# arielgabizon/barretenberg

Measured on AMD Instinct MI355X. Metric: BN254 G1 MSM points/sec at n=2^20 (Fr NTT elems/sec in 'ntt'), higher is better.
Workload: dtype u32x9 (256-bit Montgomery, 29-bit limbs)

## Files before the change

### barretenberg_amd/bbgpu.py

```python
import ctypes as C
import os
import subprocess

import numpy as np

try:
    import torch
except Exception:
    torch = None

HERE = os.path.dirname(os.path.abspath(__file__))
os.environ.setdefault("GPU_MAX_HW_QUEUES", "16")
u64p = C.POINTER(C.c_uint64)

NTT_KINDS = {
    "fft": 0,
    "ifft": 1,
    "coset_fft": 2,
    "coset_ifft": 3,
    "fft_with_constant": 4,
    "ifft_with_constant": 5,
    "coset_fft_with_constant": 6,
}

C_ABI_SYMBOLS = [
    "bbgpu_init", "bbgpu_shutdown", "bbgpu_device_count", "bbgpu_last_error", "bbgpu_version", "bbgpu_ntt",
    "bbgpu_ntt_device", "bbgpu_ntt_device_batch", "bbgpu_srs_register", "bbgpu_srs_release", "bbgpu_srs_generate", "bbgpu_srs_generate_range", "bbgpu_set_precompute",
    "bbgpu_srs_num_windows", "bbgpu_transcript_read_g1", "bbgpu_transcript_write", "bbgpu_msm_g1", "bbgpu_msm_g1_plain",
    "bbgpu_msm_g1_batch", "bbgpu_msm_num_windows", "bbgpu_msm_g1_device", "bbgpu_msm_g1_device_async", "bbgpu_msm_g1_device_rows_async", "bbgpu_msm_g1_device_buckets_async", "bbgpu_srs_has_window_tables", "bbgpu_msm_g1_wait",
    "bbgpu_msm_g1_device_batch_async", "bbgpu_msm_g1_batch_wait",
    "bbgpu_g1_sum", "bbgpu_last_timing", "bbgpu_set_host_thresholds", "bbgpu_srs_cache_stats", "bbgpu_set_table_share", "bbgpu_set_point_share", "bbgpu_selftest_field", "bbgpu_selftest_g1",
    "bbgpu_set_timing",
    "bbgpu_fr_evaluate_device", "bbgpu_fr_batch_invert_device", "bbgpu_fr_product_scan_device", "bbgpu_fr_mul_device",
    "bbgpu_kate_opening_device", "bbgpu_lagrange_l1_fft_device", "bbgpu_divide_by_pseudo_vanishing_device",
    "bbgpu_permutation_lagrange_base_device",
    "bbgpu_fr_evaluate", "bbgpu_kate_opening", "bbgpu_lagrange_l1_fft", "bbgpu_divide_by_pseudo_vanishing", "bbgpu_lagrange_evaluations",
    "bbgpu_generate_point_table",
    "bbgpu_plonk_prover_create", "bbgpu_plonk_prover_set_witness", "bbgpu_plonk_construct_proof", "bbgpu_plonk_preprocess", "bbgpu_plonk_last_challenges",
    "bbgpu_plonk_last_timing", "bbgpu_plonk_prover_destroy", "bbgpu_plonk_challenges_from_proof",
    "bbgpu_plonk_construct_proof_batch", "bbgpu_plonk_batch_challenges", "bbgpu_plonk_last_batch_timing",
    "bbgpu_host_msm_g1", "bbgpu_host_ntt", "bbgpu_host_fr_evaluate", "bbgpu_host_kate_opening", "bbgpu_host_lagrange_l1_fft",
    "bbgpu_host_divide_by_pseudo_vanishing", "bbgpu_memory_stats", "bbgpu_fault_inject", "bbgpu_fault_stats", "bbgpu_srs_set_validate",
    "bbgpu_init_devices", "bbgpu_num_contexts", "bbgpu_memory_stats_context",
    "bbgpu_plonk_check_witness", "bbgpu_plonk_check_witness_batch", "bbgpu_plonk_set_witness_check", "bbgpu_plonk_last_witness_report",
    "bbgpu_host_plonk_check_witness",
    "bbgpu_plonk_prover_set_wire_map", "bbgpu_plonk_prover_set_witness_from", "bbgpu_plonk_construct_proof_batch_from",
# ... 240 lines not shown
        arr = (MsmJob * len(jobs))()
        for j, (pts, sc, n) in zip(arr, jobs):
            j.points, j.scalars, j.num_elements = _ptr(pts), _ptr(sc), n
        self._chk(self.lib.bbgpu_msm_g1_batch(arr, len(jobs)))
        return [np.array(list(j.output), dtype=np.uint64) for j in arr]

    def msm_num_windows(self, n):
        return int(self.lib.bbgpu_msm_num_windows(n))

    def srs_num_windows(self, handle, n):
        return self._chk(self.lib.bbgpu_srs_num_windows(handle, n))

    def set_host_thresholds(self, msm_max_points, ntt_max_elements):
        self.lib.bbgpu_set_host_thresholds(int(msm_max_points), int(ntt_max_elements))

    def set_table_share(self, rank, world):
        self.lib.bbgpu_set_table_share(int(rank), int(world))

    def set_point_share(self, world):
        self.lib.bbgpu_set_point_share(int(world))

    def set_precompute(self, on=True):
        self.lib.bbgpu_set_precompute(1 if on else 0)

    def msm_device(self, handle, d_scalars_ptr, n, offset=0, window_begin=0, window_end=None, stream=None):
        if window_end is None:
            window_end = self.srs_num_windows(handle, n)
        out = np.zeros(12, dtype=np.uint64)
        self._chk(self.lib.bbgpu_msm_g1_device(handle, offset, C.c_void_p(d_scalars_ptr), n, window_begin, window_end,
                                               _ptr(out), C.c_void_p(stream or 0)))
# ... 106 lines not shown
```

### barretenberg_amd/csrc/bbgpu_internal.h

```cpp
#pragma once
#include <hip/hip_runtime.h>
#include <stddef.h>
#include <stdint.h>

#include <mutex>

#include "../../include/bbgpu.h"

namespace bbgpu {

void set_error(const char* fmt, ...);

hipError_t dev_malloc(void** p, size_t bytes);
hipError_t dev_free(void* p);
hipError_t h2d_async(void* dst, const void* src, size_t bytes, hipStream_t st);
hipError_t d2h_async(void* dst, const void* src, size_t bytes, hipStream_t st);
hipError_t launch_check();
struct DevBuf {
    void* p = nullptr;
    DevBuf() = default;
    DevBuf(const DevBuf&) = delete;
    DevBuf& operator=(const DevBuf&) = delete;
    ~DevBuf() { if (p) (void)dev_free(p); }
    template <class T> T* as() const { return static_cast<T*>(p); }
// ... 12 lines not shown
    int count = 0;
    float ms[8];
};
struct MsmWorkspace {
    uint8_t* base = nullptr;
    size_t cap = 0;
    void* h_out = nullptr;
    static size_t bytes_needed(size_t n, int c, int nw, int ng = 0);
    int ensure(size_t bytes);
    void release();
};
struct MsmPiece {
    uint32_t c = 0, nw = 0, wb = 0, hbits = 0, lbits = 0;
    uint32_t hout_group = 0;
    bool trivial = false;
};
struct AccRing {
    static constexpr int SIZE = 8;
    hipEvent_t end[SIZE] = {};
    uint64_t seq = 0;
    void release();
};
constexpr int MSM_MAX_JOBS = 4;
constexpr int MSM_MAX_PIECES = 64;
constexpr uint32_t MSM_HOUT_GROUPS = 256;
struct MsmSlot {
    MsmWorkspace ws;
    MsmPiece piece[MSM_MAX_PIECES];
    int npieces = 0;
    bool append = false;
    int helper = -1;
    bool is_helper = false;
    bool reserved = false;
    hipStream_t stream = nullptr;
    hipEvent_t done = nullptr;
    hipEvent_t ev[8] = { nullptr, nullptr, nullptr, nullptr, nullptr, nullptr, nullptr, nullptr };
    bool pending = false, trivial = false, timed = false, timed_light = false;
    size_t n = 0;
    uint32_t jobs = 1;
    uint64_t acc_seq = 0;
    AccRing* acc_ring = nullptr;
    bool throughput = false;
    void release();
};
int msm_choose_c(size_t n);
int msm_num_windows(int c);
int msm_issue(MsmSlot& S, const uint32_t* d_srs, const uint32_t* d_tab, size_t tab_stride, int tab_c, const uint64_t* d_scalars, size_t n, int wb,
              int we, hipStream_t st, int want_timing);
int msm_issue_batch(MsmSlot& S, const uint32_t* d_srs, const uint32_t* d_tab, size_t tab_stride, int tab_c, const uint64_t* const* d_scalars_v, int jobs,
                    size_t n, int wb, int we, hipStream_t st, int want_timing, uint32_t row_i0 = 0, uint32_t row_i1 = 0xffffffffu, uint32_t brow0 = 0,
                    uint32_t brow1 = 0xffffffffu);
int msm_issue_buckets(MsmSlot& S, const uint32_t* d_srs, const uint32_t* d_tab, size_t tab_stride, int tab_c, const uint64_t* d_scalars, size_t n,
                      uint32_t share, uint32_t share_count, hipStream_t st, int want_timing);
int msm_issue_rows(MsmSlot& S, const uint32_t* d_srs, const uint32_t* d_tab, size_t tab_stride, int tab_c, const uint64_t* d_scalars, size_t n,
                   uint64_t row_begin, uint64_t row_end, hipStream_t st, int want_timing);
int msm_finish_batch(MsmSlot& S, host::Xyzz* results, MsmTiming* timing);
int srs_build_table(const uint32_t* d_srs, size_t n, int c, int num_windows, int w_begin, int w_end, uint32_t** d_alloc_out, uint32_t** d_tab_out, hipStream_t st);
int msm_finish(MsmSlot& S, host::Xyzz* result, MsmTiming* timing);
int srs_upload(const uint64_t* host_table, size_t n, uint32_t** d_srs_out, hipStream_t st, size_t stride_bytes = 128);
int srs_upload_into(const uint64_t* host_table, size_t n, uint32_t* d_raw, uint32_t* d_srs, hipStream_t st, size_t stride_bytes);
int srs_generate(const uint64_t* x_mont256, size_t first, size_t n, uint32_t** d_srs_out, uint64_t* host_table_out, hipStream_t st);

int host_to_device(void* d_dst, const void* h_src, size_t bytes, hipStream_t st);
int device_to_host_sync(void* h_dst, const void* d_src, size_t bytes, hipStream_t st, bool* touched = nullptr);
void host_stage_release();
int bind_calling_thread();

std::mutex& plonk_mutex();
void plonk_release_all_locked();
uint64_t plonk_lane_bytes();

// ... 2 lines not shown
```

### barretenberg_amd/csrc/capi.hip

```cpp
#include <hip/hip_runtime.h>

#include <algorithm>
#include <mutex>
#include <stdarg.h>
#include <stdio.h>
#include <stdlib.h>
#include <string.h>
#include <time.h>
#include <atomic>
#include <condition_variable>
#include <exception>
#include <functional>
#include <thread>
#include <unordered_map>
#include <vector>

#include "bbgpu_internal.h"
#include "host_g1.hpp"
#include "host_g2.hpp"
#include "host_small.hpp"
#include "host_fallback.hpp"
#include "host_copy_pool.hpp"
#include "multi_plan.hpp"
#include "poly.h"
// ... 786 lines not shown
    SrsEntry& e = ctx().srs[idx];
    if (trace_srs()) fprintf(stderr, "bbgpu srs: full check: contents of %p differ from the resident copy\n", (const void*)e.host_ptr);
    if (e.auto_registered) free_entry(e);
    else e.stale_for_host = true;
}

int log2_exact(size_t n)
{
    if (n == 0 || (n & (n - 1))) return -1;
    int l = 0;
    while (((size_t)1 << l) < n) l++;
    return l;
}

int msm_host_ptrs_once(const uint64_t* scalars, const uint64_t* points, size_t n, host::Xyzz* out, bool plain, bool* stale);
int msm_host_ptrs_sum(const uint64_t* scalars, const uint64_t* points, size_t n, host::Xyzz* out, bool plain = false)
{
    bool stale = false;
    int rc = msm_host_ptrs_once(scalars, points, n, out, plain, &stale);
    if (stale) rc = msm_host_ptrs_once(scalars, points, n, out, plain, &stale);
    return rc;
}
int msm_host_ptrs(const uint64_t* scalars, const uint64_t* points, size_t n, uint64_t out[12], bool plain = false)
{
    host::Xyzz res;
    const int rc = msm_host_ptrs_sum(scalars, points, n, &res, plain);
    if (rc == BBGPU_OK) host::g1_to_normalised(res, out);
    return rc;
}
int msm_host_ptrs_once(const uint64_t* scalars, const uint64_t* points, size_t n, host::Xyzz* out, bool plain, bool* stale)
// ... 68 lines not shown
    const SrsEntry& e = is_transient ? transient : ctx().srs[idx];
    static const size_t split_env = [] { const char* v = getenv("BBGPU_HOST_MSM_SPLIT"); return v ? (size_t)std::max(1, atoi(v)) : (size_t)0; }();
    struct Range { size_t o, len; };
    std::vector<Range> ranges;
    {
        PointPiece pc[MAX_POINT_PIECES];
        const int np = split_pieces(e, off, n, pc, MAX_POINT_PIECES);
        if (np < 0) {
            if (is_transient && !small_once) (void)dev_free(transient.d_srs);
            set_error("MSM of %zu points spans more than %d table segments", n, MAX_POINT_PIECES);
            return BBGPU_ERR_SIZE;
        }
        if (np > 1) {
            for (int k = 0; k < np; k++) ranges.push_back(Range{ pc[k].first, pc[k].len });
        } else {
            const size_t parts = ns < 2 ? 1 : (split_env ? split_env : (n >= ((size_t)1 << 19) ? 2 : 1));
            const size_t base = parts == 2 ? ((n * 3 / 8) & ~(size_t)7) : n / parts;
            for (size_t k = 0; k < parts; k++) {
                const size_t o = k * base, len = (k + 1 == parts) ? n - o : base;
                if (len) ranges.push_back(Range{ o, len });
            }
        }
    }
    size_t max_len = 0;
    for (const auto& r : ranges) max_len = std::max(max_len, r.len);
    const double q1 = tr ? now_ms() : 0;
    uint64_t** stage[2] = { &ctx().d_stage, &ctx().d_stage2 };
    size_t* cap[2] = { &ctx().stage_cap, &ctx().stage2_cap };
    host::Xyzz res = host::g1_infinity();
    int rc = BBGPU_OK;
    size_t issued = 0, finished = 0;
    auto finish = [&](size_t k) -> int {
        host::Xyzz part;
        int r = finish_ticket(sl[k % (size_t)ns], &part, k + 1 == ranges.size() ? &ctx().last : nullptr);
        finished = k + 1;
        if (r == BBGPU_OK) res = host::g1_add(res, part);
        return r;
    };
    for (size_t k = 0; k < ranges.size() && rc == BBGPU_OK; k++) {
        const size_t w = k % (size_t)ns;
        if (k >= (size_t)ns) rc = finish(k - (size_t)ns);
        MsmSlot& S = ctx().slot[sl[w]];
        if (rc == BBGPU_OK) rc = grow(stage[w], cap[w], max_len * 32);
        if (rc == BBGPU_OK) rc = host_to_device(*stage[w], scalars + ranges[k].o * 4, ranges[k].len * 32, S.stream);
        if (rc == BBGPU_OK) rc = issue_on_entry(sl[w], e, off + ranges[k].o, *stage[w], ranges[k].len, 0, entry_windows(e, ranges[k].len), S.stream);
        if (rc == BBGPU_OK) issued = k + 1;
    }
    const double q2 = tr ? now_ms() : 0;
    if (rc == BBGPU_OK && full_check && !(bg.posted ? full_check_join(bg) : contents_match_full(ctx().srs[idx], off, points, n))) {
        for (int k = 0; k < ns; k++) drain_ticket(sl[k]);
        srs_mark_stale(idx);
        *stale = true;
        return BBGPU_OK;
    }
    while (rc == BBGPU_OK && finished < issued) rc = finish(finished);
    if (rc != BBGPU_OK) {
        char keep[sizeof(g_err)];
        memcpy(keep, g_err, sizeof(keep));
        for (int k = 0; k < ns; k++) drain_ticket(sl[k]);
        memcpy(g_err, keep, sizeof(keep));
    }
    const double q3 = tr ? now_ms() : 0;
    if (is_transient && !small_once) (void)dev_free(transient.d_srs);
    if (rc) return rc;
    *out = res;
    if (tr) fprintf(stderr, "bbgpu msm n=%zu: table %.3f, upload + issue %.3f, wait + host sums %.3f, free %.3f ms\n", n, q1 - q0, q2 - q1, q3 - q2, now_ms() - q3);
    return BBGPU_OK;
}

struct MultiWorker {
    std::mutex mu;
    std::condition_variable cv;
    std::function<int()> job;
    bool busy = false, stop = false;
    int rc = BBGPU_OK;
    std::exception_ptr ex;
    char err[sizeof(g_err)] = "";
    std::thread th;
    explicit MultiWorker(int k) { th = std::thread([this, k] { loop(k); }); }
    void loop(int k)
// ... 918 lines not shown
{
    std::lock_guard<std::recursive_mutex> lk(g_mu);
    return msm_host_ptrs(scalars, points, n, out, true);
}

void bbgpu_set_host_thresholds(int msm_max_points, int ntt_max_elements)
{
    std::lock_guard<std::recursive_mutex> lk(g_mu);
    for (auto& C : g_ctxs) {
        C.host_env_read = true;
        C.host_msm_max = msm_max_points < 0 ? 0 : msm_max_points;
        C.host_ntt_max = ntt_max_elements < 0 ? 0 : std::min(64, ntt_max_elements);
    }
}

static int msm_g1_batch_once(bbgpu_msm_job* jobs, size_t num_jobs, bool* stale, host::Xyzz* sums);
static int msm_g1_batch_run(bbgpu_msm_job* jobs, size_t num_jobs, host::Xyzz* sums)
{
    bool stale = false;
    int rc = msm_g1_batch_once(jobs, num_jobs, &stale, sums);
    if (stale) rc = msm_g1_batch_once(jobs, num_jobs, &stale, sums);
    return rc;
}
static bool batch_one_by_one(size_t n, int* sl)
{
    return n == 0 || n <= (size_t)ctx().host_msm_max || n > ((size_t)1 << 20) || free_slots(sl, 2) < 2;
}
static int msm_g1_batch_split(bbgpu_msm_job* jobs, size_t num_jobs, const multi::Slice* sl, int m)
{
    if (num_jobs == 0) return BBGPU_OK;
// ... 359 lines not shown
```

### barretenberg_amd/csrc/msm.hip

```cpp
#include <hip/hip_runtime.h>

#include <algorithm>
#include <mutex>
#include <stdint.h>
#include <stdio.h>
#include <stdlib.h>
#include <string.h>
#include <vector>

#include "bbgpu_internal.h"
#include "g1.hpp"
#include "g1_quad.hpp"
#include "host_g1.hpp"

namespace bbgpu {

using Fr = FrP;
#define FRONT_PRIO() __builtin_amdgcn_s_setprio(2)
constexpr int TAIL_PRIO = 3;
constexpr int SCALAR_BITS = 254;
constexpr int MSM_MAX_C = 16;
constexpr int MSM_THREADS = 256;

__device__ __forceinline__ void ld8(const uint32_t* p, uint32_t (&w)[8])
// ... 821 lines not shown
        if (t < half) {
            Xyzz q, r;
#pragma unroll
            for (int i = 0; i < NL; i++) {
                q.x.d[i] = sh[(0 * NL + i) * STRIDE + t];
                q.y.d[i] = sh[(1 * NL + i) * STRIDE + t];
                q.zz.d[i] = sh[(2 * NL + i) * STRIDE + t];
                q.zzz.d[i] = sh[(3 * NL + i) * STRIDE + t];
            }
            add(r, acc, q);
            acc = r;
        }
        __syncthreads();
    }
}
__global__ void __launch_bounds__(MSM_THREADS) TAIL_OCC msm_merge_kernel(const uint32_t* __restrict__ gstart, const uint32_t* __restrict__ partials,
                                                              uint32_t* __restrict__ buckets, uint32_t* __restrict__ heavy, uint32_t bucket_begin, uint32_t total_buckets,
                                                              uint32_t ch, uint32_t MERGE_LIGHT, uint32_t logG)
{
    __builtin_amdgcn_s_setprio(TAIL_PRIO);
    const uint32_t t = blockIdx.x * blockDim.x + threadIdx.x;
    const uint32_t G = 1u << logG, b = bucket_begin + (t >> logG), j = t & (G - 1);
    if (b >= total_buckets) return;
    const uint32_t s = gstart[b], e = gstart[b + 1];
    Xyzz acc;
    set_infinity(acc);
    if (e > s) {
        const uint32_t t0 = s / ch, t1 = (e - 1) / ch;
        if (t1 - t0 >= MERGE_LIGHT) {
            if (j == 0) heavy[HEAVY_IDS + atomicAdd(&heavy[0], 1u)] = b;
            return;
        }
        for (uint32_t k = t0 + j; k <= t1; k += G) {
            Xyzz q, r;
            load_raw(q, partials + (size_t)(b + k) * RAW_WORDS);
            add(r, acc, q);
            acc = r;
        }
    }
    for (uint32_t off = G >> 1; off >= 1; off >>= 1) {
        const Xyzz o = shfl_down_xyzz(acc, off);
        if (j < off) {
            Xyzz r;
            add(r, acc, o);
            acc = r;
        }
    }
    if (j == 0) {
        uint32_t o[32];
        store_xyzz(o, acc);
        st32(buckets + (size_t)b * 32, o);
    }
}
__global__ void __launch_bounds__(MSM_THREADS) TAIL_OCC msm_merge_heavy_kernel(const uint32_t* __restrict__ gstart, const uint32_t* __restrict__ partials,
                                                                    uint32_t* __restrict__ buckets, uint32_t* __restrict__ heavy, uint32_t ch, uint32_t* __restrict__ hpart)
{
    __builtin_amdgcn_s_setprio(TAIL_PRIO);
    __shared__ uint32_t sh[FOLD_LDS_WORDS];
    __shared__ uint32_t last_flag;
    const uint32_t count = heavy[0];
    const uint32_t K = count ? gridDim.x / count : 0;
    if (K < 2) {
        for (uint32_t item = blockIdx.x; item < count; item += gridDim.x) {
            const uint32_t b = heavy[HEAVY_IDS + item];
            const uint32_t s = gstart[b], e = gstart[b + 1];
            const uint32_t t0 = s / ch, t1 = (e - 1) / ch;
            Xyzz acc;
            set_infinity(acc);
            for (uint32_t t = t0 + threadIdx.x; t <= t1; t += MSM_THREADS) {
                Xyzz q, r;
                load_raw(q, partials + (size_t)(b + t) * RAW_WORDS);
                add(r, acc, q);
                acc = r;
            }
            __syncthreads();
            wg_tree_sum(acc, sh, MSM_THREADS, threadIdx.x);
            if (threadIdx.x == 0) {
                uint32_t o[32];
                store_xyzz(o, acc);
                st32(buckets + (size_t)b * 32, o);
            }
        }
        return;
    }
    const uint32_t item = blockIdx.x / K, sub = blockIdx.x - item * K;
    if (item >= count) return;
    const uint32_t b = heavy[HEAVY_IDS + item];
    const uint32_t s = gstart[b], e = gstart[b + 1];
    const uint32_t t0 = s / ch, t1 = (e - 1) / ch, total = t1 - t0 + 1;
    const uint32_t lo = t0 + (uint32_t)(((uint64_t)total * sub) / K), hi = t0 + (uint32_t)(((uint64_t)total * (sub + 1)) / K);
    Xyzz acc;
    set_infinity(acc);
    for (uint32_t t = lo + threadIdx.x; t < hi; t += MSM_THREADS) {
// ... 5 lines not shown
    wg_tree_sum(acc, sh, MSM_THREADS, threadIdx.x);
    if (threadIdx.x == 0) {
        store_raw(hpart + (size_t)blockIdx.x * RAW_WORDS, acc);
        __threadfence();
        last_flag = (atomicAdd(&heavy[1 + item], 1u) == K - 1) ? 1u : 0u;
    }
    __syncthreads();
    if (!last_flag) return;
    __threadfence();
    set_infinity(acc);
    if (threadIdx.x < K) load_raw(acc, hpart + (size_t)(item * K + threadIdx.x) * RAW_WORDS);
    __syncthreads();
    wg_tree_sum(acc, sh, MSM_THREADS, threadIdx.x);
    if (threadIdx.x == 0) {
        uint32_t o[32];
        store_xyzz(o, acc);
        st32(buckets + (size_t)b * 32, o);
    }
}

__device__ __forceinline__ uint32_t insert_one_bit(uint32_t m, uint32_t k)
{
    return ((m >> k) << (k + 1)) | (1u << k) | (m & ((1u << k) - 1));
}
constexpr int QFOLD_T = 256;
__device__ __forceinline__ FqN quad_load(const uint32_t* point32, uint32_t l)
{
    const uint4* q = reinterpret_cast<const uint4*>(point32 + 8 * l);
    const uint4 a = q[0], b = q[1];
    const uint32_t w[8] = { a.x, a.y, a.z, a.w, b.x, b.y, b.z, b.w };
// ... 36 lines not shown
            for (int i = 0; i < NL; i++) o.d[i] = __shfl_down(acc.d[i], off * 4);
            if (qd < off) acc = quad_add(acc, o, l);
        }
    }
    return acc;
}
__device__ __forceinline__ void quad_store8(uint32_t* dst8, const uint32_t (&w)[8])
{
    uint4* q = reinterpret_cast<uint4*>(dst8);
    q[0] = make_uint4(w[0], w[1], w[2], w[3]);
    q[1] = make_uint4(w[4], w[5], w[6], w[7]);
}

__global__ void __launch_bounds__(MSM_THREADS) TAIL_OCC msm_merge_quad_kernel(const uint32_t* __restrict__ gstart, const uint32_t* __restrict__ partials,
                                                                   uint32_t* __restrict__ buckets, uint32_t* __restrict__ heavy, uint32_t bucket_begin, uint32_t total_buckets,
                                                                   uint32_t ch, uint32_t MERGE_LIGHT, uint32_t logQ)
{
    __builtin_amdgcn_s_setprio(TAIL_PRIO);
    const uint32_t t = blockIdx.x * blockDim.x + threadIdx.x, l = t & 3, quad = t >> 2;
    const uint32_t Q = 1u << logQ, b = bucket_begin + (quad >> logQ), j = quad & (Q - 1);
    if (b >= total_buckets) return;
    const uint32_t s = gstart[b], e = gstart[b + 1];
    FqN acc = quad_zero();
    if (e > s) {
        const uint32_t t0 = s / ch, t1 = (e - 1) / ch;
        if (t1 - t0 >= MERGE_LIGHT) {
            if (j == 0 && l == 0) heavy[HEAVY_IDS + atomicAdd(&heavy[0], 1u)] = b;
            return;
        }
        uint32_t k = t0 + j;
        if (k <= t1) {
// ... 8 lines not shown
                for (int i = 0; i < NL; i++) q.d[i] = src[i];
            }
            while (k <= t1) {
                FqN qn = quad_zero();
                const uint32_t kn = k + Q;
                if (kn <= t1) {
                    src = partials + (size_t)(b + kn) * RAW_WORDS + NL * l;
#pragma unroll
                    for (int i = 0; i < NL; i++) qn.d[i] = src[i];
                }
                acc = quad_add(acc, q, l);
                q = qn;
                k = kn;
            }
        }
    }
    for (uint32_t off = Q >> 1; off >= 1; off >>= 1) {
        FqN o;
#pragma unroll
        for (int i = 0; i < NL; i++) o.d[i] = __shfl_down(acc.d[i], off * 4);
        if (j < off) acc = quad_add(acc, o, l);
    }
    if (j == 0) {
        uint32_t w[8];
        to_canonical(acc, w);
        quad_store8(buckets + (size_t)b * 32 + 8 * l, w);
    }
}

__global__ void __launch_bounds__(QFOLD_T) TAIL_OCC msm_rowcol_quad_kernel(const uint32_t* __restrict__ buckets, uint32_t* __restrict__ R, uint32_t* __restrict__ Cc,
                                                                  uint32_t H, uint32_t L, uint32_t* __restrict__ zero_out, uint32_t zero_words, uint32_t r0, uint32_t rows)
{
    __builtin_amdgcn_s_setprio(TAIL_PRIO);
    __shared__ uint32_t sh[(QFOLD_T / 64) * 4 * NL];
    const uint32_t g = blockIdx.y, t = threadIdx.x, nb = H * L, l = t & 3, quad = t >> 2;
    if (zero_out) {
        const uint32_t gid = (g * gridDim.x + blockIdx.x) * blockDim.x + t, all = gridDim.y * gridDim.x * blockDim.x;
        for (uint32_t i = gid; i < zero_words; i += all) zero_out[i] = 0;
    }
// ... 195 lines not shown
    if ((uint64_t)P.slices * 4096 > n) P.slices = std::max<uint32_t>(1, (uint32_t)(n / 4096));
    P.slice_len = (uint32_t)((n + P.slices - 1) / P.slices);
    return P;
}

struct MsmCarve {
    size_t digits, signs, histA, histB, binstart, bintot, tmp_entries, gstart, totals, heavy, sorted, partials, buckets, arena, segs, end;
    size_t chunks_cap, histB_bytes;
};
static MsmCarve carve(const MsmPlan& P, size_t n, size_t nw, size_t ng)
{
    auto al = [](size_t x) { return (x + 255) & ~(size_t)255; };
    MsmCarve L;
    size_t p = 0;
    const size_t wmax = std::max<size_t>(P.W, nw);
    L.digits = p;      p += al(wmax * n * 2);
    L.signs = p;       p += al(wmax * ((n + 63) / 64) * 8);
    L.histA = p;       p += al(nw * P.slices * 1024 * 4);
    L.histB_bytes = (uint64_t)n * nw >= ((uint64_t)1 << 21) ? (size_t)MSM_MAX_JOBS * 1024 * SORTB_MAX_PARTS * 128 * 4 : 0;
    L.histB = p;       p += al(L.histB_bytes);
    L.binstart = p;    p += al(nw * 1024 * 4 + 256);
    L.bintot = p;      p += al(nw * 1024 * 4 + 256);
    L.tmp_entries = p; p += al(nw * n * 4);
    L.gstart = p;      p += al((ng * P.nb + 2) * 4);
    L.totals = p;      p += al(nw * 8 + 512);
    L.heavy = p;       p += al((ng * P.nb + HEAVY_IDS) * 4 + 256 + (size_t)HEAVY_WGS * RAW_WORDS * 4);
    L.sorted = p;      p += al(nw * n * 4);
    L.chunks_cap = (n * nw + min_chunk(n * nw) - 1) / min_chunk(n * nw) + 1;
    L.partials = p;    p += al((ng * P.nb + L.chunks_cap) * RAW_WORDS * 4);
    L.buckets = p;     p += al(ng * P.nb * 128);
    L.arena = p;       p += al(arena_points(P, (uint32_t)ng) * 128);
    L.segs = p;        p += al(seg_points(P, (uint32_t)ng) * 128);
    L.end = p;
    return L;
}
size_t MsmWorkspace::bytes_needed(size_t n, int c, int nw, int ng)
{
    return carve(make_plan(n, c), n, (size_t)nw, (size_t)(ng > 0 ? ng : nw)).end;
}

int MsmWorkspace::ensure(size_t bytes)
{
    if (bytes <= cap) return BBGPU_OK;
    if (base) (void)dev_free(base);
    base = nullptr;
    cap = 0;
    HIPCHK(dev_malloc((void**)&base, bytes));
    cap = bytes;
    return BBGPU_OK;
}
void MsmWorkspace::release()
{
    if (base) (void)dev_free(base);
// ... 45 lines not shown
void AccRing::release()
{
    if (seq)
        for (auto& e : end) {
            if (e) (void)hipEventDestroy(e);
            e = nullptr;
        }
    seq = 0;
}
int msm_issue_batch(MsmSlot& S, const uint32_t* d_srs, const uint32_t* d_tab, size_t tab_stride, int tab_c, const uint64_t* const* d_scalars_v, int jobs,
                    size_t n, int wb, int we, hipStream_t st, int want_timing, uint32_t row_i0, uint32_t row_i1, uint32_t brow0, uint32_t brow1)
{
    MsmWorkspace& ws = S.ws;
    const bool append = S.append && S.pending && S.npieces > 0;
    S.append = false;
    if (append && (S.jobs != (uint32_t)jobs || S.npieces >= MSM_MAX_PIECES)) {
        set_error("internal: MSM piece %d does not continue the MSM on this slot", S.npieces);
        return BBGPU_ERR_STATE;
    }
    if (!append) {
        S.jobs = (uint32_t)jobs;
        S.n = n;
        S.pending = false;
        S.timed = false;
        S.npieces = 0;
    } else {
        S.n += n;
    }
    MsmPiece& PC = S.piece[S.npieces];
    PC = MsmPiece{};
// ... 8 lines not shown
    const bool table = d_tab != nullptr;
    const int c = table ? tab_c : msm_choose_c(n);
    const MsmPlan P = make_plan(n, c);
    if (wb < 0 || we > (int)P.W || wb >= we) return BBGPU_ERR_ARG;
    if (row_i1 > n) row_i1 = (uint32_t)n;
    if ((row_i0 != 0 || row_i1 != n) && (!table || jobs != 1 || row_i0 >= n || (we - wb == 1 && row_i0 >= row_i1))) return BBGPU_ERR_ARG;
    if (jobs < 1 || jobs > MSM_MAX_JOBS || (jobs > 1 && (!table || wb != 0 || we != (int)P.W))) {
        set_error("batched MSM: 1..%d jobs, window tables and the full window range required", MSM_MAX_JOBS);
        return BBGPU_ERR_ARG;
    }
    const uint32_t BH = 1u << P.hbits, BL = 1u << P.lbits;
    if (brow1 > BH) brow1 = BH;
    const bool bshare = brow0 != 0 || brow1 != BH;
    if (bshare && (!table || jobs != 1 || brow0 >= brow1 || wb != 0 || we != (int)P.W || row_i0 != 0 || row_i1 != n)) return BBGPU_ERR_ARG;
    const uint32_t blo = brow0 * BL, bcnt = (brow1 - brow0) * BL;
    const uint32_t nw1 = (uint32_t)(we - wb);
    const uint32_t nw = nw1 * (uint32_t)jobs;
    const uint32_t G = table ? (uint32_t)jobs : nw1;
    const uint32_t wpg = table ? nw1 : 1u;
    uint32_t sort_lb = P.sort_lb, sort_bins = P.sort_bins;
    if (table) {
        uint32_t want_bins = 512;
        while (sort_bins < want_bins && sort_lb > 3) { sort_lb--; sort_bins <<= 1; }
    }
    uint32_t slices = table ? std::max<uint32_t>(1, P.slices * nw1 / 2) : P.slices;
    if (table && jobs == 1) {
        const uint32_t by_cap = (uint32_t)(((uint64_t)nw * P.slices * 1024) / ((uint64_t)G * sort_bins));
        const uint32_t want = std::min<uint32_t>(std::min<uint32_t>(208, (uint32_t)(n / 2048)), by_cap);
        slices = std::max(slices, want);
    }
    const uint32_t slice_len = (uint32_t)((n + slices - 1) / slices);
    const uint32_t idx_stride = table ? (uint32_t)tab_stride : 0u;
    const uint32_t* points = table ? d_tab : d_srs;
    PC.c = P.c; PC.nw = G; PC.wb = table ? 0u : (uint32_t)wb; PC.hbits = P.hbits; PC.lbits = P.lbits;
    if (PC.hout_group + G > MSM_HOUT_GROUPS) {
        set_error("MSM in %d pieces of %u bucket sets: the result array holds %u", S.npieces + 1, G, MSM_HOUT_GROUPS);
        return BBGPU_ERR_SIZE;
    }
    int rc = ws.ensure(MsmWorkspace::bytes_needed(n, c, (int)nw, (int)G));
    if (rc) return rc;
    if (!ws.h_out) HIPCHK(hipHostMalloc((void**)&ws.h_out, (size_t)MSM_HOUT_GROUPS * 64 * 128));
    if (!S.done) HIPCHK(hipEventCreateWithFlags(&S.done, hipEventDisableTiming));

    const MsmCarve LY = carve(P, n, nw, G);
    if (LY.end > ws.cap) {
        set_error("internal: MSM workspace of %zu bytes, layout needs %zu (n=%zu c=%d nw=%u)", ws.cap, LY.end, n, c, nw);
        return BBGPU_ERR_STATE;
    }
    uint8_t* const p = ws.base;
    void* digits = (void*)(p + LY.digits);
    unsigned long long* signs = (unsigned long long*)(p + LY.signs);
    uint32_t* histA = (uint32_t*)(p + LY.histA);
    uint32_t* histB = (uint32_t*)(p + LY.histB);
    uint32_t* binstart = (uint32_t*)(p + LY.binstart);
    uint32_t* bintot = (uint32_t*)(p + LY.bintot);
    uint32_t* tmp_entries = (uint32_t*)(p + LY.tmp_entries);
    uint32_t* gstart = (uint32_t*)(p + LY.gstart);
    uint32_t* totals = (uint32_t*)(p + LY.totals);
    uint32_t* bases = totals + nw;
    uint32_t* heavy = (uint32_t*)(p + LY.heavy);
    uint32_t* sorted = (uint32_t*)(p + LY.sorted);
    uint32_t* partials = (uint32_t*)(p + LY.partials);
    uint32_t* buckets = (uint32_t*)(p + LY.buckets);
    uint32_t* scratch = (uint32_t*)(p + LY.arena);
    if ((uint64_t)G * slices * sort_bins > (uint64_t)nw * P.slices * 1024 || sort_bins > 1024 ||
        (size_t)G * ((size_t)(1u << P.hbits) + (size_t)(1u << P.lbits)) + 64 > arena_points(P, G)) {
        set_error("internal: MSM launch shape exceeds the workspace layout");
        return BBGPU_ERR_STATE;
    }

    hipEvent_t* ev = S.ev;
    const bool tm = want_timing == 1, tm_acc = want_timing != 0;
    S.timed_light = want_timing == 2;
    if (tm_acc) {
        if (!S.ev[0])
            for (int i = 0; i < 8; i++) HIPCHK(hipEventCreate(&S.ev[i]));
        if (tm) HIPCHK(hipEventRecord(ev[0], st));
        S.timed = true;
// ... 38 lines not shown
    ch = std::max(ch, min_chunk((uint64_t)n * nw));
    if (tp && ch < TP_MIN_CHUNK)
        ch = std::max(ch, std::min<uint32_t>(TP_MIN_CHUNK, (uint32_t)(m_expected / (acc_capacity_lanes() / ACC_WG_PER_CU))));
    const uint32_t avg_partials = (uint32_t)(m_expected / ((uint64_t)merge_buckets * ch)) + 1;
    uint32_t logG = 0;
    while ((1u << logG) < avg_partials && logG < 6 && ((uint64_t)merge_buckets << (logG + 1)) <= ((uint64_t)1 << 16)) logG++;
    const uint32_t merge_light = std::max(6u, 8u << logG);
    const uint32_t max_chunks = (uint32_t)(((uint64_t)n * nw + ch - 1) / ch);
    msm_accumulate_kernel<<<(max_chunks + MSM_THREADS - 1) / MSM_THREADS, MSM_THREADS, ACC_LDS_RESERVE, st>>>(points, sorted, gstart, partials, total_buckets, ch, 0, heavy);
    if (tm_acc) {
        HIPCHK(hipEventRecord(ev[3], st));
        if (int rc = acc_ring_record(S, st)) return rc;
    } else {
        S.acc_seq = 0;
    }
    if ((uint64_t)n * nw <= ((uint64_t)1 << 21)) {
        uint32_t logQ = 0;
        while ((2u << logQ) < avg_partials && logQ < 4 && ((uint64_t)merge_buckets << (logQ + 3)) <= ((uint64_t)1 << 17)) logQ++;
        msm_merge_quad_kernel<<<(uint32_t)((((uint64_t)merge_buckets << (logQ + 2)) + MSM_THREADS - 1) / MSM_THREADS), MSM_THREADS, 0, st>>>(gstart, partials, buckets, heavy, blo, blo + merge_buckets, ch,
                                                                                                                                  std::max(32u, 8u << logQ), logQ);
    } else msm_merge_kernel<<<(uint32_t)((((uint64_t)merge_buckets << logG) + MSM_THREADS - 1) / MSM_THREADS), MSM_THREADS, 0, st>>>(gstart, partials, buckets, heavy,
                                                                                                                     blo, blo + merge_buckets, ch, merge_light, logG);
    msm_merge_heavy_kernel<<<HEAVY_WGS, MSM_THREADS, 0, st>>>(gstart, partials, buckets, heavy, ch, heavy + (((size_t)G * P.nb + HEAVY_IDS + 63) & ~(size_t)63));
    if (tm) HIPCHK(hipEventRecord(ev[4], st));

    const uint32_t H = 1u << P.hbits, L = 1u << P.lbits;
    {
        uint32_t* Rr = scratch;
        uint32_t* Cc = scratch + (size_t)G * H * 32;
        uint32_t* const dest = (uint32_t*)ws.h_out + (size_t)PC.hout_group * 64 * 32;
        const uint32_t zero_words = G * 64 * 32;
        if (!bshare && rowcol_two_step(P) && (tp || jobs > 1)) {
            uint32_t* segs = (uint32_t*)(p + LY.segs);
            const uint32_t seg_lanes = 2 * (H * L / ROWCOL_SEG);
            msm_rowcol_seg_kernel<<<dim3((seg_lanes + MSM_THREADS - 1) / MSM_THREADS, G), MSM_THREADS, 0, st>>>(buckets, segs, H, L, dest, zero_words);
            msm_segsum_quad_kernel<<<dim3(H + L, G), 64, 0, st>>>(segs, Rr, Cc, H, L);
        } else msm_rowcol_quad_kernel<<<dim3((bshare ? brow1 - brow0 : H) + L, G), QFOLD_T, 0, st>>>(buckets, Rr, Cc, H, L, dest, zero_words, bshare ? brow0 : 0u,
                                                                                                  bshare ? brow1 - brow0 : H);
        if (tm) HIPCHK(hipEventRecord(ev[5], st));
        msm_final_quad_kernel<<<dim3(1 + P.hbits + P.lbits, G), QFOLD_T, 0, st>>>(Rr, Cc, dest, P.hbits, P.lbits);
        if (tm) HIPCHK(hipEventRecord(ev[6], st));
    }
    HIPCHK(hipEventRecord(S.done, st));
    HIPCHK(launch_check());
    S.npieces++;
    S.pending = true;
    return BBGPU_OK;
}

static host::Xyzz group_sum(const MsmSlot& S, const MsmPiece& PC, uint32_t w)
{
    auto pt = [&](uint32_t slot) {
        host::Xyzz q;
        memcpy(&q, (const uint8_t*)S.ws.h_out + ((size_t)(PC.hout_group + w) * 64 + slot) * 128, 128);
        return q;
    };
    host::Xyzz rs = host::g1_infinity();
    for (int k = (int)PC.hbits - 1; k >= 0; --k) rs = host::g1_add(host::g1_dbl(rs), pt(1 + k));
    for (uint32_t k = 0; k < PC.lbits; k++) rs = host::g1_dbl(rs);
    host::Xyzz cs = host::g1_infinity();
    for (int k = (int)PC.lbits - 1; k >= 0; --k) cs = host::g1_add(host::g1_dbl(cs), pt(32 + k));
    return host::g1_add(host::g1_add(rs, cs), pt(0));
}
static int finish_timing(MsmSlot& S, MsmTiming* timing)
{
    if (S.timed && timing) {
        float ms;
        timing->count = 0;
        if (S.timed_light) {
            for (int i = 0; i < 7; i++) timing->ms[timing->count++] = 0.0f;
            HIPCHK(hipEventElapsedTime(&ms, S.ev[2], S.ev[3]));
            timing->ms[3] = ms;
        } else {
            HIPCHK(hipEventElapsedTime(&ms, S.ev[0], S.ev[6]));
            timing->ms[timing->count++] = ms;
            for (int i = 0; i < 6; i++) {
                HIPCHK(hipEventElapsedTime(&ms, S.ev[i], S.ev[i + 1]));
                timing->ms[timing->count++] = ms;
            }
        }
        float exec = timing->ms[3];
        const AccRing* R = S.acc_ring;
        if (R && S.acc_seq > 1 && R->seq - (S.acc_seq - 1) < (uint64_t)ACC_RING &&
            hipEventElapsedTime(&ms, R->end[(S.acc_seq - 1) % ACC_RING], R->end[S.acc_seq % ACC_RING]) == hipSuccess && ms > 0.0f && ms < exec)
            exec = ms;
        (void)hipGetLastError();
        timing->ms[timing->count++] = exec;
    }
    return BBGPU_OK;
}
int msm_finish(MsmSlot& S, host::Xyzz* result, MsmTiming* timing)
{
    *result = host::g1_infinity();
    if (!S.pending) return BBGPU_ERR_STATE;
    if (S.jobs > 1) return BBGPU_ERR_STATE;
    S.pending = false;
    bool waited = false;
    host::Xyzz total = host::g1_infinity();
    for (int pi = 0; pi < S.npieces; pi++) {
        const MsmPiece& PC = S.piece[pi];
        if (PC.trivial) continue;
        if (!waited) HIPCHK(hipEventSynchronize(S.done));
        waited = true;
        host::Xyzz acc = host::g1_infinity();
        for (int w = (int)PC.nw - 1; w >= 0; --w) {
            for (uint32_t k = 0; k < PC.c; k++) acc = host::g1_dbl(acc);
            acc = host::g1_add(acc, group_sum(S, PC, (uint32_t)w));
        }
        for (uint32_t k = 0; k < PC.c * PC.wb; k++) acc = host::g1_dbl(acc);
        total = host::g1_add(total, acc);
    }
    *result = total;
    if (!waited) return BBGPU_OK;
    return finish_timing(S, timing);
}
int msm_finish_batch(MsmSlot& S, host::Xyzz* results, MsmTiming* timing)
{
    if (S.jobs <= 1) return msm_finish(S, results, timing);
// ... 5 lines not shown
        const MsmPiece& PC = S.piece[pi];
        if (PC.trivial) continue;
        if (!waited) HIPCHK(hipEventSynchronize(S.done));
        waited = true;
        for (uint32_t j = 0; j < S.jobs; j++) results[j] = host::g1_add(results[j], group_sum(S, PC, j));
    }
    if (!waited) return BBGPU_OK;
    return finish_timing(S, timing);
}

void MsmSlot::release()
{
    ws.release();
    if (done) (void)hipEventDestroy(done);
    done = nullptr;
    for (auto& e : ev) {
        if (e) (void)hipEventDestroy(e);
        e = nullptr;
    }
    if (stream) (void)hipStreamDestroy(stream);
    stream = nullptr;
    pending = false;
    npieces = 0;
    helper = -1;
    is_helper = append = false;
}

int srs_upload(const uint64_t* host_table, size_t n, uint32_t** d_srs_out, hipStream_t st, size_t stride_bytes)
{
    DevBuf tab, srs;
// ... 62 lines not shown
```

### include/bbgpu.h

```cpp
#ifndef BBGPU_H
#define BBGPU_H

#include <stddef.h>
#include <stdint.h>

#ifdef __cplusplus
extern "C" {
#endif

enum {
    BBGPU_OK = 0,
    BBGPU_ERR_HIP = -1,
    BBGPU_ERR_SIZE = -2,
    BBGPU_ERR_ARG = -3,
    BBGPU_ERR_STATE = -4,
    BBGPU_ERR_LOST = -5,
    BBGPU_ERR_WITNESS = -6
};

typedef enum {
    BBGPU_FFT = 0,
    BBGPU_IFFT = 1,
    BBGPU_COSET_FFT = 2,
    BBGPU_COSET_IFFT = 3,
// ... 47 lines not shown
int bbgpu_srs_set_validate(int srs_handle, int full);
void bbgpu_set_precompute(int enabled);
void bbgpu_set_table_share(int rank, int world);
void bbgpu_set_point_share(int world);
int bbgpu_srs_num_windows(int srs_handle, size_t n);
int bbgpu_srs_release(int handle);
int bbgpu_srs_cache_stats(int* live_entries, int* auto_entries, uint64_t* auto_bytes);
int bbgpu_transcript_read_g1(const char* path, size_t degree, uint64_t* points_endo_table_out);
int bbgpu_transcript_write(const char* path, const uint64_t* points_endo_table, size_t degree, const uint64_t x_mont[4]);
int bbgpu_srs_generate(const uint64_t* x_mont, size_t n, uint64_t* host_endo_table_out);
int bbgpu_srs_generate_range(const uint64_t* x_mont, size_t first, size_t n, uint64_t* host_endo_table_out);

int bbgpu_msm_g1(const uint64_t* scalars, const uint64_t* points_endo_table, size_t n, uint64_t out[12]);
int bbgpu_msm_g1_plain(const uint64_t* scalars, const uint64_t* points, size_t n, uint64_t out[12]);
void bbgpu_set_host_thresholds(int msm_max_points, int ntt_max_elements);

typedef struct {
    const uint64_t* points;
    const uint64_t* scalars;
    size_t num_elements;
    uint64_t _pad;
    uint64_t output[12];
} bbgpu_msm_job;
int bbgpu_msm_g1_batch(bbgpu_msm_job* jobs, size_t num_jobs);

int bbgpu_msm_num_windows(size_t n);
int bbgpu_msm_g1_device(int srs_handle, size_t offset, const uint64_t* d_scalars, size_t n, int window_begin,
                        int window_end, uint64_t out[12], void* hip_stream);
int bbgpu_msm_g1_device_async(int srs_handle, size_t offset, const uint64_t* d_scalars, size_t n, int window_begin,
                              int window_end, void* hip_stream);
// ... 130 lines not shown
```

Before: 921.9 million.

## Share bucket accumulators across host MSM ranges and run the tail once

When a host-pointer MSM is split into several ranges with window tables, all ranges now accumulate into one shared bucket array. Each later range's merge kernels add into the existing bucket values, ordered by events across streams, and only the last range runs the bucket reduction tail and host window sum. This removes the repeated per-range tail reduction and host combination work. The cost is cross-stream serialization of the merge stages, extra loads in the carry merge, and added API knobs for range count and first-range fraction.

Result: no change. 921.2 million (-0.1%).

```diff
diff --git a/barretenberg_amd/bbgpu.py b/barretenberg_amd/bbgpu.py
--- a/barretenberg_amd/bbgpu.py
+++ b/barretenberg_amd/bbgpu.py
@@ -29,7 +29,7 @@
     "bbgpu_srs_num_windows", "bbgpu_transcript_read_g1", "bbgpu_transcript_write", "bbgpu_msm_g1", "bbgpu_msm_g1_plain",
     "bbgpu_msm_g1_batch", "bbgpu_msm_num_windows", "bbgpu_msm_g1_device", "bbgpu_msm_g1_device_async", "bbgpu_msm_g1_device_rows_async", "bbgpu_msm_g1_device_buckets_async", "bbgpu_srs_has_window_tables", "bbgpu_msm_g1_wait",
     "bbgpu_msm_g1_device_batch_async", "bbgpu_msm_g1_batch_wait",
-    "bbgpu_g1_sum", "bbgpu_last_timing", "bbgpu_set_host_thresholds", "bbgpu_srs_cache_stats", "bbgpu_set_table_share", "bbgpu_set_point_share", "bbgpu_selftest_field", "bbgpu_selftest_g1",
+    "bbgpu_g1_sum", "bbgpu_last_timing", "bbgpu_set_host_thresholds", "bbgpu_set_host_msm_ranges", "bbgpu_srs_cache_stats", "bbgpu_set_table_share", "bbgpu_set_point_share", "bbgpu_selftest_field", "bbgpu_selftest_g1",
     "bbgpu_set_timing",
     "bbgpu_fr_evaluate_device", "bbgpu_fr_batch_invert_device", "bbgpu_fr_product_scan_device", "bbgpu_fr_mul_device",
     "bbgpu_kate_opening_device", "bbgpu_lagrange_l1_fft_device", "bbgpu_divide_by_pseudo_vanishing_device",
@@ -300,6 +300,9 @@
     def set_host_thresholds(self, msm_max_points, ntt_max_elements):
         self.lib.bbgpu_set_host_thresholds(int(msm_max_points), int(ntt_max_elements))
 
+    def set_host_msm_ranges(self, parts=0, first_permille=0):
+        self.lib.bbgpu_set_host_msm_ranges(int(parts), int(first_permille))
+
     def set_table_share(self, rank, world):
         self.lib.bbgpu_set_table_share(int(rank), int(world))
 
diff --git a/barretenberg_amd/csrc/bbgpu_internal.h b/barretenberg_amd/csrc/bbgpu_internal.h
--- a/barretenberg_amd/csrc/bbgpu_internal.h
+++ b/barretenberg_amd/csrc/bbgpu_internal.h
@@ -50,6 +50,7 @@
     uint32_t c = 0, nw = 0, wb = 0, hbits = 0, lbits = 0;
     uint32_t hout_group = 0;
     bool trivial = false;
+    bool no_tail = false;
 };
 struct AccRing {
     static constexpr int SIZE = 8;
@@ -77,6 +78,12 @@
     uint64_t acc_seq = 0;
     AccRing* acc_ring = nullptr;
     bool throughput = false;
+    uint32_t* shared_buckets = nullptr;
+    bool carry_in = false;
+    bool no_tail = false;
+    hipEvent_t merge_after = nullptr;
+    hipEvent_t merged = nullptr;
+    int timed_stages = 6;
     void release();
 };
 int msm_choose_c(size_t n);
@@ -91,6 +98,7 @@
 int msm_issue_rows(MsmSlot& S, const uint32_t* d_srs, const uint32_t* d_tab, size_t tab_stride, int tab_c, const uint64_t* d_scalars, size_t n,
                    uint64_t row_begin, uint64_t row_end, hipStream_t st, int want_timing);
 int msm_finish_batch(MsmSlot& S, host::Xyzz* results, MsmTiming* timing);
+uint32_t* msm_workspace_buckets(const MsmSlot& S);
 int srs_build_table(const uint32_t* d_srs, size_t n, int c, int num_windows, int w_begin, int w_end, uint32_t** d_alloc_out, uint32_t** d_tab_out, hipStream_t st);
 int msm_finish(MsmSlot& S, host::Xyzz* result, MsmTiming* timing);
 int srs_upload(const uint64_t* host_table, size_t n, uint32_t** d_srs_out, hipStream_t st, size_t stride_bytes = 128);
diff --git a/barretenberg_amd/csrc/capi.hip b/barretenberg_amd/csrc/capi.hip
--- a/barretenberg_amd/csrc/capi.hip
+++ b/barretenberg_amd/csrc/capi.hip
@@ -824,6 +824,8 @@
 }
 
 int msm_host_ptrs_once(const uint64_t* scalars, const uint64_t* points, size_t n, host::Xyzz* out, bool plain, bool* stale);
+constexpr size_t HOST_MSM_PARTS = 2, HOST_MSM_FIRST_PERMILLE = 375;
+int g_host_msm_parts = 0, g_host_msm_first_permille = 0;
 int msm_host_ptrs_sum(const uint64_t* scalars, const uint64_t* points, size_t n, host::Xyzz* out, bool plain = false)
 {
     bool stale = false;
@@ -922,11 +924,16 @@
         if (np > 1) {
             for (int k = 0; k < np; k++) ranges.push_back(Range{ pc[k].first, pc[k].len });
         } else {
-            const size_t parts = ns < 2 ? 1 : (split_env ? split_env : (n >= ((size_t)1 << 19) ? 2 : 1));
-            const size_t base = parts == 2 ? ((n * 3 / 8) & ~(size_t)7) : n / parts;
-            for (size_t k = 0; k < parts; k++) {
-                const size_t o = k * base, len = (k + 1 == parts) ? n - o : base;
-                if (len) ranges.push_back(Range{ o, len });
+            const size_t forced = is_transient ? 0 : (g_host_msm_parts > 0 ? (size_t)g_host_msm_parts : split_env);
+            size_t parts = ns < 2 ? 1 : (forced ? forced : (n >= ((size_t)1 << 19) ? HOST_MSM_PARTS : 1));
+            const size_t permille = (!is_transient && g_host_msm_first_permille > 0) ? (size_t)g_host_msm_first_permille : (parts == HOST_MSM_PARTS ? HOST_MSM_FIRST_PERMILLE : 1000 / parts);
+            size_t first = parts > 1 ? ((n * std::min<size_t>(permille, 999) / 1000) & ~(size_t)7) : n;
+            size_t base = parts > 1 ? (((n - first) / (parts - 1)) & ~(size_t)7) : 0;
+            if (parts > 1 && (first == 0 || base == 0)) { first = n; parts = 1; }
+            for (size_t k = 0, o = 0; k < parts; k++) {
+                const size_t len = k == 0 ? first : (k + 1 == parts ? n - o : base);
+                ranges.push_back(Range{ o, len });
+                o += len;
             }
         }
     }
@@ -937,12 +944,31 @@
     size_t* cap[2] = { &ctx().stage_cap, &ctx().stage2_cap };
     host::Xyzz res = host::g1_infinity();
     int rc = BBGPU_OK;
+    const bool shared = e.has_tab() && ranges.size() > 1;
+    uint32_t* shared_buckets = nullptr;
+    if (shared) {
+        for (int w = 0; w < ns && rc == BBGPU_OK; w++) {
+            size_t need = 0;
+            for (size_t k = (size_t)w; k < ranges.size(); k += (size_t)ns) need = std::max(need, MsmWorkspace::bytes_needed(ranges[k].len, e.tab_c, e.tab_W, 1));
+            if (need) rc = ctx().slot[sl[w]].ws.ensure(need);
+        }
+        if (rc == BBGPU_OK) shared_buckets = msm_workspace_buckets(ctx().slot[sl[0]]);
+    }
     size_t issued = 0, finished = 0;
+    MsmTiming call_timing;
+    for (float& v : call_timing.ms) v = 0.0f;
     auto finish = [&](size_t k) -> int {
         host::Xyzz part;
-        int r = finish_ticket(sl[k % (size_t)ns], &part, k + 1 == ranges.size() ? &ctx().last : nullptr);
+        MsmTiming t;
+        int r = finish_ticket(sl[k % (size_t)ns], &part, &t);
         finished = k + 1;
-        if (r == BBGPU_OK) res = host::g1_add(res, part);
+        if (r != BBGPU_OK) return r;
+        if (!shared) res = host::g1_add(res, part);
+        else if (k + 1 == ranges.size()) res = part;
+        if (t.count > 0) {
+            call_timing.count = t.count;
+            for (int i = 0; i < t.count; i++) call_timing.ms[i] += t.ms[i];
+        }
         return r;
     };
     for (size_t k = 0; k < ranges.size() && rc == BBGPU_OK; k++) {
@@ -951,7 +977,16 @@
         MsmSlot& S = ctx().slot[sl[w]];
         if (rc == BBGPU_OK) rc = grow(stage[w], cap[w], max_len * 32);
         if (rc == BBGPU_OK) rc = host_to_device(*stage[w], scalars + ranges[k].o * 4, ranges[k].len * 32, S.stream);
+        if (rc == BBGPU_OK && shared) {
+            S.shared_buckets = shared_buckets;
+            S.carry_in = k > 0;
+            S.no_tail = k + 1 < ranges.size();
+            S.merge_after = (k > 0 && ns > 1) ? ctx().slot[sl[(k - 1) % (size_t)ns]].merged : nullptr;
+        }
         if (rc == BBGPU_OK) rc = issue_on_entry(sl[w], e, off + ranges[k].o, *stage[w], ranges[k].len, 0, entry_windows(e, ranges[k].len), S.stream);
+        S.shared_buckets = nullptr;
+        S.carry_in = S.no_tail = false;
+        S.merge_after = nullptr;
         if (rc == BBGPU_OK) issued = k + 1;
     }
     const double q2 = tr ? now_ms() : 0;
@@ -966,12 +1001,15 @@
         char keep[sizeof(g_err)];
         memcpy(keep, g_err, sizeof(keep));
         for (int k = 0; k < ns; k++) drain_ticket(sl[k]);
+        if (shared)
+            for (int k = 0; k < ns; k++) (void)hipStreamSynchronize(ctx().slot[sl[k]].stream);
         memcpy(g_err, keep, sizeof(keep));
     }
     const double q3 = tr ? now_ms() : 0;
     if (is_transient && !small_once) (void)dev_free(transient.d_srs);
     if (rc) return rc;
     *out = res;
+    if (call_timing.count > 0) ctx().last = call_timing;
     if (tr) fprintf(stderr, "bbgpu msm n=%zu: table %.3f, upload + issue %.3f, wait + host sums %.3f, free %.3f ms\n", n, q1 - q0, q2 - q1, q3 - q2, now_ms() - q3);
     return BBGPU_OK;
 }
@@ -1920,6 +1958,13 @@
     }
 }
 
+void bbgpu_set_host_msm_ranges(int parts, int first_permille)
+{
+    std::lock_guard<std::recursive_mutex> lk(g_mu);
+    g_host_msm_parts = parts > 0 ? std::min(parts, MSM_MAX_PIECES) : 0;
+    g_host_msm_first_permille = first_permille > 0 ? std::min(first_permille, 999) : 0;
+}
+
 static int msm_g1_batch_once(bbgpu_msm_job* jobs, size_t num_jobs, bool* stale, host::Xyzz* sums);
 static int msm_g1_batch_run(bbgpu_msm_job* jobs, size_t num_jobs, host::Xyzz* sums)
 {
diff --git a/barretenberg_amd/csrc/msm.hip b/barretenberg_amd/csrc/msm.hip
--- a/barretenberg_amd/csrc/msm.hip
+++ b/barretenberg_amd/csrc/msm.hip
@@ -859,9 +859,18 @@
         __syncthreads();
     }
 }
+__device__ __forceinline__ void add_stored(Xyzz& acc, const uint32_t* point32)
+{
+    uint32_t w[32];
+    ld32(point32, w);
+    Xyzz q, r;
+    load_xyzz(q, w);
+    add(r, acc, q);
+    acc = r;
+}
 __global__ void __launch_bounds__(MSM_THREADS) TAIL_OCC msm_merge_kernel(const uint32_t* __restrict__ gstart, const uint32_t* __restrict__ partials,
                                                               uint32_t* __restrict__ buckets, uint32_t* __restrict__ heavy, uint32_t bucket_begin, uint32_t total_buckets,
-                                                              uint32_t ch, uint32_t MERGE_LIGHT, uint32_t logG)
+                                                              uint32_t ch, uint32_t MERGE_LIGHT, uint32_t logG, uint32_t carry)
 {
     __builtin_amdgcn_s_setprio(TAIL_PRIO);
     const uint32_t t = blockIdx.x * blockDim.x + threadIdx.x;
@@ -882,7 +891,7 @@
             add(r, acc, q);
             acc = r;
         }
-    }
+    } else if (carry) return;
     for (uint32_t off = G >> 1; off >= 1; off >>= 1) {
         const Xyzz o = shfl_down_xyzz(acc, off);
         if (j < off) {
@@ -893,12 +902,14 @@
     }
     if (j == 0) {
         uint32_t o[32];
+        if (carry) add_stored(acc, buckets + (size_t)b * 32);
         store_xyzz(o, acc);
         st32(buckets + (size_t)b * 32, o);
     }
 }
 __global__ void __launch_bounds__(MSM_THREADS) TAIL_OCC msm_merge_heavy_kernel(const uint32_t* __restrict__ gstart, const uint32_t* __restrict__ partials,
-                                                                    uint32_t* __restrict__ buckets, uint32_t* __restrict__ heavy, uint32_t ch, uint32_t* __restrict__ hpart)
+                                                                    uint32_t* __restrict__ buckets, uint32_t* __restrict__ heavy, uint32_t ch, uint32_t* __restrict__ hpart,
+                                                                    uint32_t carry)
 {
     __builtin_amdgcn_s_setprio(TAIL_PRIO);
     __shared__ uint32_t sh[FOLD_LDS_WORDS];
@@ -922,6 +933,7 @@
             wg_tree_sum(acc, sh, MSM_THREADS, threadIdx.x);
             if (threadIdx.x == 0) {
                 uint32_t o[32];
+                if (carry) add_stored(acc, buckets + (size_t)b * 32);
                 store_xyzz(o, acc);
                 st32(buckets + (size_t)b * 32, o);
             }
@@ -957,6 +969,7 @@
     wg_tree_sum(acc, sh, MSM_THREADS, threadIdx.x);
     if (threadIdx.x == 0) {
         uint32_t o[32];
+        if (carry) add_stored(acc, buckets + (size_t)b * 32);
         store_xyzz(o, acc);
         st32(buckets + (size_t)b * 32, o);
     }
@@ -1023,7 +1036,7 @@
 
 __global__ void __launch_bounds__(MSM_THREADS) TAIL_OCC msm_merge_quad_kernel(const uint32_t* __restrict__ gstart, const uint32_t* __restrict__ partials,
                                                                    uint32_t* __restrict__ buckets, uint32_t* __restrict__ heavy, uint32_t bucket_begin, uint32_t total_buckets,
-                                                                   uint32_t ch, uint32_t MERGE_LIGHT, uint32_t logQ)
+                                                                   uint32_t ch, uint32_t MERGE_LIGHT, uint32_t logQ, uint32_t carry)
 {
     __builtin_amdgcn_s_setprio(TAIL_PRIO);
     const uint32_t t = blockIdx.x * blockDim.x + threadIdx.x, l = t & 3, quad = t >> 2;
@@ -1062,7 +1075,7 @@
                 k = kn;
             }
         }
-    }
+    } else if (carry) return;
     for (uint32_t off = Q >> 1; off >= 1; off >>= 1) {
         FqN o;
 #pragma unroll
@@ -1071,6 +1084,7 @@
     }
     if (j == 0) {
         uint32_t w[8];
+        if (carry) acc = quad_add(acc, quad_load(buckets + (size_t)b * 32, l), l);
         to_canonical(acc, w);
         quad_store8(buckets + (size_t)b * 32 + 8 * l, w);
     }
@@ -1296,6 +1310,7 @@
     MsmCarve L;
     size_t p = 0;
     const size_t wmax = std::max<size_t>(P.W, nw);
+    L.buckets = p;     p += al(ng * P.nb * 128);
     L.digits = p;      p += al(wmax * n * 2);
     L.signs = p;       p += al(wmax * ((n + 63) / 64) * 8);
     L.histA = p;       p += al(nw * P.slices * 1024 * 4);
@@ -1310,7 +1325,6 @@
     L.sorted = p;      p += al(nw * n * 4);
     L.chunks_cap = (n * nw + min_chunk(n * nw) - 1) / min_chunk(n * nw) + 1;
     L.partials = p;    p += al((ng * P.nb + L.chunks_cap) * RAW_WORDS * 4);
-    L.buckets = p;     p += al(ng * P.nb * 128);
     L.arena = p;       p += al(arena_points(P, (uint32_t)ng) * 128);
     L.segs = p;        p += al(seg_points(P, (uint32_t)ng) * 128);
     L.end = p;
@@ -1319,6 +1333,11 @@
 size_t MsmWorkspace::bytes_needed(size_t n, int c, int nw, int ng)
 {
     return carve(make_plan(n, c), n, (size_t)nw, (size_t)(ng > 0 ? ng : nw)).end;
+}
+
+uint32_t* msm_workspace_buckets(const MsmSlot& S)
+{
+    return (uint32_t*)S.ws.base;
 }
 
 int MsmWorkspace::ensure(size_t bytes)
@@ -1394,6 +1413,12 @@
     MsmWorkspace& ws = S.ws;
     const bool append = S.append && S.pending && S.npieces > 0;
     S.append = false;
+    uint32_t* const shared_buckets = S.shared_buckets;
+    const bool carry_in = S.carry_in, no_tail = S.no_tail;
+    const hipEvent_t merge_after = S.merge_after;
+    S.shared_buckets = nullptr;
+    S.carry_in = S.no_tail = false;
+    S.merge_after = nullptr;
     if (append && (S.jobs != (uint32_t)jobs || S.npieces >= MSM_MAX_PIECES)) {
         set_error("internal: MSM piece %d does not continue the MSM on this slot", S.npieces);
         return BBGPU_ERR_STATE;
@@ -1432,6 +1457,11 @@
     const bool bshare = brow0 != 0 || brow1 != BH;
     if (bshare && (!table || jobs != 1 || brow0 >= brow1 || wb != 0 || we != (int)P.W || row_i0 != 0 || row_i1 != n)) return BBGPU_ERR_ARG;
     const uint32_t blo = brow0 * BL, bcnt = (brow1 - brow0) * BL;
+    const bool sharing = shared_buckets || carry_in || no_tail;
+    if (sharing && (!shared_buckets || !table || jobs != 1 || bshare || append || wb != 0 || we != (int)P.W || row_i0 != 0 || row_i1 != n)) {
+        set_error("internal: shared buckets need window tables, one job and the whole window range");
+        return BBGPU_ERR_STATE;
+    }
     const uint32_t nw1 = (uint32_t)(we - wb);
     const uint32_t nw = nw1 * (uint32_t)jobs;
     const uint32_t G = table ? (uint32_t)jobs : nw1;
@@ -1451,6 +1481,7 @@
     const uint32_t idx_stride = table ? (uint32_t)tab_stride : 0u;
     const uint32_t* points = table ? d_tab : d_srs;
     PC.c = P.c; PC.nw = G; PC.wb = table ? 0u : (uint32_t)wb; PC.hbits = P.hbits; PC.lbits = P.lbits;
+    PC.no_tail = no_tail;
     if (PC.hout_group + G > MSM_HOUT_GROUPS) {
         set_error("MSM in %d pieces of %u bucket sets: the result array holds %u", S.npieces + 1, G, MSM_HOUT_GROUPS);
         return BBGPU_ERR_SIZE;
@@ -1479,7 +1510,7 @@
     uint32_t* heavy = (uint32_t*)(p + LY.heavy);
     uint32_t* sorted = (uint32_t*)(p + LY.sorted);
     uint32_t* partials = (uint32_t*)(p + LY.partials);
-    uint32_t* buckets = (uint32_t*)(p + LY.buckets);
+    uint32_t* buckets = shared_buckets ? shared_buckets : (uint32_t*)(p + LY.buckets);
     uint32_t* scratch = (uint32_t*)(p + LY.arena);
     if ((uint64_t)G * slices * sort_bins > (uint64_t)nw * P.slices * 1024 || sort_bins > 1024 ||
         (size_t)G * ((size_t)(1u << P.hbits) + (size_t)(1u << P.lbits)) + 64 > arena_points(P, G)) {
@@ -1548,18 +1579,26 @@
     } else {
         S.acc_seq = 0;
     }
+    const uint32_t carry = carry_in ? 1u : 0u;
+    if (merge_after) HIPCHK(hipStreamWaitEvent(st, merge_after, 0));
     if ((uint64_t)n * nw <= ((uint64_t)1 << 21)) {
         uint32_t logQ = 0;
         while ((2u << logQ) < avg_partials && logQ < 4 && ((uint64_t)merge_buckets << (logQ + 3)) <= ((uint64_t)1 << 17)) logQ++;
         msm_merge_quad_kernel<<<(uint32_t)((((uint64_t)merge_buckets << (logQ + 2)) + MSM_THREADS - 1) / MSM_THREADS), MSM_THREADS, 0, st>>>(gstart, partials, buckets, heavy, blo, blo + merge_buckets, ch,
-                                                                                                                                  std::max(32u, 8u << logQ), logQ);
+                                                                                                                                  std::max(32u, 8u << logQ), logQ, carry);
     } else msm_merge_kernel<<<(uint32_t)((((uint64_t)merge_buckets << logG) + MSM_THREADS - 1) / MSM_THREADS), MSM_THREADS, 0, st>>>(gstart, partials, buckets, heavy,
-                                                                                                                     blo, blo + merge_buckets, ch, merge_light, logG);
-    msm_merge_heavy_kernel<<<HEAVY_WGS, MSM_THREADS, 0, st>>>(gstart, partials, buckets, heavy, ch, heavy + (((size_t)G * P.nb + HEAVY_IDS + 63) & ~(size_t)63));
+                                                                                                                     blo, blo + merge_buckets, ch, merge_light, logG, carry);
+    msm_merge_heavy_kernel<<<HEAVY_WGS, MSM_THREADS, 0, st>>>(gstart, partials, buckets, heavy, ch, heavy + (((size_t)G * P.nb + HEAVY_IDS + 63) & ~(size_t)63), carry);
     if (tm) HIPCHK(hipEventRecord(ev[4], st));
+    S.timed_stages = no_tail ? 4 : 6;
+    if (sharing) {
+        if (!S.merged) HIPCHK(hipEventCreateWithFlags(&S.merged, hipEventDisableTiming));
+        HIPCHK(hipEventRecord(S.merged, st));
+    }
+    HIPCHK(launch_check());
 
     const uint32_t H = 1u << P.hbits, L = 1u << P.lbits;
-    {
+    if (!no_tail) {
         uint32_t* Rr = scratch;
         uint32_t* Cc = scratch + (size_t)G * H * 32;
         uint32_t* const dest = (uint32_t*)ws.h_out + (size_t)PC.hout_group * 64 * 32;
@@ -1574,9 +1613,9 @@
         if (tm) HIPCHK(hipEventRecord(ev[5], st));
         msm_final_quad_kernel<<<dim3(1 + P.hbits + P.lbits, G), QFOLD_T, 0, st>>>(Rr, Cc, dest, P.hbits, P.lbits);
         if (tm) HIPCHK(hipEventRecord(ev[6], st));
+        HIPCHK(launch_check());
     }
     HIPCHK(hipEventRecord(S.done, st));
-    HIPCHK(launch_check());
     S.npieces++;
     S.pending = true;
     return BBGPU_OK;
@@ -1606,10 +1645,12 @@
             HIPCHK(hipEventElapsedTime(&ms, S.ev[2], S.ev[3]));
             timing->ms[3] = ms;
         } else {
-            HIPCHK(hipEventElapsedTime(&ms, S.ev[0], S.ev[6]));
+            const int last = S.timed_stages;
+            HIPCHK(hipEventElapsedTime(&ms, S.ev[0], S.ev[last]));
             timing->ms[timing->count++] = ms;
             for (int i = 0; i < 6; i++) {
-                HIPCHK(hipEventElapsedTime(&ms, S.ev[i], S.ev[i + 1]));
+                ms = 0.0f;
+                if (i < last) HIPCHK(hipEventElapsedTime(&ms, S.ev[i], S.ev[i + 1]));
                 timing->ms[timing->count++] = ms;
             }
         }
@@ -1636,6 +1677,7 @@
         if (PC.trivial) continue;
         if (!waited) HIPCHK(hipEventSynchronize(S.done));
         waited = true;
+        if (PC.no_tail) continue;
         host::Xyzz acc = host::g1_infinity();
         for (int w = (int)PC.nw - 1; w >= 0; --w) {
             for (uint32_t k = 0; k < PC.c; k++) acc = host::g1_dbl(acc);
@@ -1671,6 +1713,11 @@
     ws.release();
     if (done) (void)hipEventDestroy(done);
     done = nullptr;
+    if (merged) (void)hipEventDestroy(merged);
+    merged = nullptr;
+    shared_buckets = nullptr;
+    merge_after = nullptr;
+    carry_in = no_tail = false;
     for (auto& e : ev) {
         if (e) (void)hipEventDestroy(e);
         e = nullptr;
diff --git a/include/bbgpu.h b/include/bbgpu.h
--- a/include/bbgpu.h
+++ b/include/bbgpu.h
@@ -85,6 +85,7 @@
 int bbgpu_msm_g1(const uint64_t* scalars, const uint64_t* points_endo_table, size_t n, uint64_t out[12]);
 int bbgpu_msm_g1_plain(const uint64_t* scalars, const uint64_t* points, size_t n, uint64_t out[12]);
 void bbgpu_set_host_thresholds(int msm_max_points, int ntt_max_elements);
+void bbgpu_set_host_msm_ranges(int parts, int first_permille);
 
 typedef struct {
     const uint64_t* points;
```
